# danieljfarrell/pvtrace

Hardware: AMD Instinct MI355X
Metric: photons/sec on 5x5x1 cm Lumogen-F-Red LSC (higher is better)
Workload: dtype f64

## Files before the change

### __graft_entry__.py

```python
import os
import subprocess
import sys

ROOT = os.path.dirname(os.path.abspath(__file__))
CSRC = os.path.join(ROOT, "pvtrace_amd", "csrc")
LIB = os.path.join(CSRC, "libpvtrace_hip.so")
HIPCC_FLAGS = [
    "--offload-arch=gfx950", "-O3", "-std=c++17",
    "-ffp-contract=off", "-fno-fast-math",
    "-munsafe-fp-atomics",
    "-mllvm", "-disable-machine-licm",
    "-fno-unroll-loops",
    "-fPIC", "-shared",
]


def _stale(target, sources):
    if not os.path.exists(target):
        return True
    t = os.path.getmtime(target)
    return any(os.path.getmtime(s) > t for s in sources if os.path.exists(s))


def build(force=False):
# ... 49 lines not shown
    for block in notes.split("- .agpr_count:")[1:]:
        name = re.search(r"\.name:\s+(\S+)", block).group(1)
        out[name] = {k: int(v) for k, v in re.findall(r"\.(sgpr_spill_count|vgpr_count|vgpr_spill_count|"
                                                      r"private_segment_fixed_size):\s+(\d+)", block)}
        out[name]["text_bytes"] = size.get(name, 0)
    return out


def code_hash(lib=LIB):
    import hashlib
    import tempfile

    llvm = "/opt/rocm/lib/llvm/bin"
    with tempfile.TemporaryDirectory() as tmp:
        fat, co, text = (os.path.join(tmp, f) for f in ("fat.bin", "k.co", "text.bin"))
        subprocess.check_call([os.path.join(llvm, "llvm-objcopy"), "-O", "binary", "--only-section=.hip_fatbin", lib, fat])
        subprocess.check_call([os.path.join(llvm, "clang-offload-bundler"), "--unbundle", "--type=o", f"--input={fat}",
                               "--targets=hipv4-amdgcn-amd-amdhsa--gfx950", f"--output={co}"],
                              stdout=subprocess.DEVNULL, stderr=subprocess.DEVNULL)
        subprocess.check_call([os.path.join(llvm, "llvm-objcopy"), "-O", "binary", "--only-section=.text", co, text])
        return hashlib.sha256(open(text, "rb").read()).hexdigest()[:16]


def check_kernel_budgets():
    meta = kernel_metadata()
    head = [m for n, m in meta.items() if "trace_kernel_w4ILb0ELi1ELi1ELb0E" in n]
    problems = []
    if head:
        m = head[0]
        if m["vgpr_count"] > 128 or m["vgpr_spill_count"] or m["private_segment_fixed_size"] > 320:
            problems.append(f"headline variant needs {m['vgpr_count']} vector registers, {m['vgpr_spill_count']} spilled, "
                            f"{m['private_segment_fixed_size']} B of scratch (budget: <= 128, 0, a call frame of <= 320 B)")
        if m["sgpr_spill_count"] > 60:
            problems.append(f"headline variant spills {m['sgpr_spill_count']} scalar registers (budget: <= 60)")
        if m["text_bytes"] > 58 * 1024:
            problems.append(f"headline variant is {m['text_bytes']} bytes of code (budget: 58 KB of the 64 KB instruction cache)")
    for n, m in meta.items():
        if "trace_kernel_gridILb0E" in n and "ELi1E" in n and (m["vgpr_spill_count"] or m["private_segment_fixed_size"] > 320):
            problems.append(f"grid-walk variant {n} uses scratch memory ({m['vgpr_spill_count']} spilled registers, "
                            f"{m['private_segment_fixed_size']} B)")
    for p in problems:
        print("=" * 100 + f"\n[build] WARNING: kernel budget exceeded -- {p}\n" + "=" * 100, file=sys.stderr)
    return problems


def smoke():
    if ROOT not in sys.path:
        sys.path.insert(0, ROOT)
    import numpy as np

    from oracle import oracle
    from pvtrace_amd.engine import _kernel, compile_scene
    from pvtrace_amd.engine.emit import emit_bundle
    from benchmarks.configs import cfg2_lsc

    scene = cfg2_lsc()
    compiled = compile_scene(scene)
    pos, dirs, wl, _ = emit_bundle(scene, 4096, seed=1)
    gpu = _kernel.trace_bundle(compiled, pos, dirs, wl, 7, 1000, 64, 0, 1, 1)
    cpu = oracle.trace_bundle(compiled, pos, dirs, wl, 7, 1000, 64, 0, 1, 1,
                              math_mode=oracle.MATH_PORTABLE)
    for key in cpu:
        if key == "rec_sums":
# ... 12 lines not shown
```

### include/pvtrace_hip.h

```cpp
#ifndef PVTRACE_HIP_H
#define PVTRACE_HIP_H

#include <stdint.h>

#ifdef __cplusplus
extern "C" {
#endif

#define PVT_ABI_VERSION 13

#define PVT_MAX_NODES 128
#define PVT_MAX_RECORDERS 256
#define PVT_MAX_HITS 512

enum {
    PVT_EV_GENERATE = 0, PVT_EV_REFLECT = 1, PVT_EV_TRANSMIT = 2, PVT_EV_ABSORB = 3,
    PVT_EV_NONRADIATIVE = 4, PVT_EV_SCATTER = 5, PVT_EV_EMIT = 6, PVT_EV_EXIT = 7,
    PVT_EV_REACT = 8, PVT_EV_KILL = 9,
    PVT_EV_DETECT = 10
};
enum { PVT_GEOM_BOX = 0, PVT_GEOM_SPHERE = 1, PVT_GEOM_CYLINDER = 2, PVT_GEOM_MESH = 3,
       PVT_GEOM_FRUSTUM = 4 };
enum { PVT_SURF_FRESNEL = 0, PVT_SURF_NULL = 1 };
enum { PVT_COMP_ABSORBER = 0, PVT_COMP_SCATTERER = 1, PVT_COMP_LUMINOPHORE = 2, PVT_COMP_REACTOR = 3 };
// ... 366 lines not shown
                           const PvtRays* rays, const PvtTraceParams* params,
                           const PvtTallies* tallies, const PvtEventLog* log,
                           const int* devices, int n_devices, double* kernel_ms);

int pvt_last_multi_reduce(void);

int pvt_shard_range(int64_t n_rays, int shard, int n_shards, int64_t align, int64_t* start, int64_t* stop);

int pvt_emit_device(PvtScene* scene, const PvtTraceParams* params, double* position,
                    double* direction, double* wavelength, void* stream);

int pvt_selftest_math(int fn, const double* x_host, double* y_host, int64_t n, int device);

int pvt_scene_counters(PvtScene* scene, uint64_t* out, int reset);

int pvt_scene_clock(PvtScene* scene, uint64_t* out);

int pvt_scene_launch_span(PvtScene* scene, void* stream, uint64_t* out);

int pvt_scene_launch_info(PvtScene* scene, int32_t* grid, int32_t* block, int32_t* lds_bytes);

enum { PVT_VARIANT_LEAN = 0, PVT_VARIANT_W4 = 1, PVT_VARIANT_GRID = 2, PVT_VARIANT_ROUGH = 3, PVT_VARIANT_MESH = 4 };
int pvt_scene_variant(PvtScene* scene);
int pvt_scene_lean_check(const PvtSceneTables* tables, const PvtIndexTables* index_tables, const PvtPhaseTables* phase_tables,
                         const PvtSurfaceTables* surface_tables, const PvtFieldTables* field_tables,
                         const PvtMapTables* map_tables, int32_t* lean);

int pvt_mesh_bvh_check(const PvtSceneTables* tables, int32_t node, int32_t* n_bvh_nodes,
                       int32_t* n_leaves, int32_t* depth);

int pvt_node_grid_plan(const PvtSceneTables* tables, int32_t* dims, double* lo, double* cell, double* guard,
                       int32_t* odd, uint64_t* masks, int64_t masks_cap);

#ifdef __cplusplus
}
#endif
#endif
```

### pvtrace_amd/csrc/pvt_trace.hip

```cpp
#include <hip/hip_runtime.h>

#include <cmath>
#include <cstdio>
#include <cstdlib>
#include <algorithm>
#include <atomic>
#include <cstring>
#include <chrono>
#include <dlfcn.h>
#include <string>
#include <thread>
#include <type_traits>
#include <mutex>
#include <vector>

#include "../../include/pvtrace_hip.h"
#include "pvt_math.h"
#include "pvt_bvh.h"

#include "pvt_trace_kernel.h"

namespace {

thread_local std::string g_error;
// ... 74 lines not shown
    };
    std::vector<Carry> carry;
    std::vector<double*> emit_pool;
    std::vector<size_t> emit_pool_bytes;
    std::vector<double*> origin_store;
    std::vector<size_t> origin_store_bytes;
    unsigned int carry_cap = 0;
    int num_cu = 0;
    int last_grid = 0, last_lds = 0;
    size_t lds_limit = 0;
    int lazy_root = 0;
    double lazy_k = 0.0;
    bool exit_observed = false;
    bool grid = false;
    int grid_dims[3] = {0, 0, 0};
    bool fuse_exit = false;
    bool hist_reads_position = false;
    bool hist_reads_counter = false;
    int origin_mask = 0;
    int counting() const { return hist_reads_counter ? 2 : d_cd ? 1 : 0; }
    bool lean_ok = false;
    bool lean_even = false;
    int last_variant = -1;
};

extern "C" {

int pvt_abi_version(void) { return PVT_ABI_VERSION; }
const char* pvt_last_error(void) { return g_error.c_str(); }

int pvt_device_count(void) {
    int n = 0;
    if (hipGetDeviceCount(&n) != hipSuccess) return 0;
    return n;
}

int pvt_scene_set_emitter(PvtScene* s, const PvtEmitterTables* e) {
    if (!s || !e || e->n_lights <= 0) return fail(PVT_ERR_INVALID, "bad emitter");
    HIP_TRY(hipSetDevice(s->device));
    std::vector<double> ed;
    std::vector<int> ei;
    EmitOff o{};
    const int Lt = e->n_lights;
    o.wl_value = push(ed, e->wl_value, Lt);
    o.pos_param = push(ed, e->pos_param, (size_t)Lt * 3);
    o.dir_param = push(ed, e->dir_param, Lt);
// ... 130 lines not shown
    const size_t small_bytes = (size_t)s->nd_small * 8 + (size_t)((s->ni_small + 1) & ~1) * 4;
    if (acc_bytes + tq_bytes + tab_bytes <= budget && !force) lp.tab = Tab::Lds;
    else if (s->meshq == 0 && acc_bytes + tq_bytes + small_bytes <= 40 * 1024 && acc_bytes + tq_bytes + small_bytes <= budget &&
             !(force && force[0] == 'g')) lp.tab = Tab::Heads;
    size_t lds = acc_bytes + tq_bytes + (lp.tab == Tab::Lds ? tab_bytes : lp.tab == Tab::Heads ? small_bytes : 0);
    lp.bins_in_lds = (lds + bins_bytes <= budget) ? 1 : 0;
    if (lp.bins_in_lds) lds += bins_bytes;
    const size_t xw = 14 + (s->n_rec <= 64 ? 1 : 4) + (record ? 1 : 0) + (s->counting() ? 2 : 0) + (s->origin_mask ? kOriginWords : 0);
    const size_t xbytes = (size_t)kXSlots * xw * 8;
    if (s->meshq == 0 && lds + xbytes <= 40 * 1024 && lds + xbytes <= lds_limit) {
        lp.xslots = kXSlots;
        lds += xbytes;
    }
    lp.total = lp.bytes = (lds + 15) & ~(size_t)15;
    if (s->meshq) {
        lp.meshq_off = (int)lp.total;
        lp.total += (size_t)s->meshq * kBlock * 4;
        lp.top_off = (int)lp.total;
        lp.total += (size_t)s->top_n * sizeof(pvt::BvhNode);
    }
    return lp;
}

struct Variant { int family; bool record; Tab tab; int seenw; bool emit, mesh, grid, even, align; };
Variant choose_variant(const PvtScene* s, const LdsPlan& lp, bool record, bool emit) {
    Variant v{};
    v.record = record; v.emit = emit; v.tab = lp.tab;
    v.seenw = s->n_rec <= 64 ? 1 : 4;
    v.mesh = s->d_bvh != nullptr;
    v.grid = lp.tab == Tab::Lds && s->lay.grid_d >= 0 && !v.mesh;
    const bool extension = s->has_frustum || s->rough_d >= 0 || s->d_fd || s->d_md || s->d_cd || s->cabs_d >= 0 || s->counting() || s->origin_mask || s->pd_d >= 0 || s->al_d >= 0;
    const bool lean = lp.tab == Tab::Lds && s->lean_ok && v.seenw == 1;
    v.align = s->al_d >= 0;
    v.family = extension ? PVT_VARIANT_ROUGH : v.mesh ? PVT_VARIANT_MESH : v.grid ? PVT_VARIANT_GRID : lean ? PVT_VARIANT_LEAN : PVT_VARIANT_W4;
    v.even = v.family == PVT_VARIANT_LEAN && s->lean_even;
    return v;
}

using Kernel = void (*)(KArgs);
template <class F> Kernel with_bool(bool b, F f) { return b ? f(std::true_type{}) : f(std::false_type{}); }
template <class F> Kernel with_tab(Tab t, F f) {
    return t == Tab::Lds ? f(std::integral_constant<int, 1>{}) : t == Tab::Heads ? f(std::integral_constant<int, 2>{}) : f(std::integral_constant<int, 0>{});
}

#ifndef PVT_DEV_VARIANTS
#define PVT_DEV_VARIANTS 0
#endif
Kernel kernel_of(const Variant& v) {
    return with_bool(v.record, [&](auto record) { return with_bool(v.emit, [&](auto emit) { return with_bool(v.seenw == 4, [&](auto wide) {
    return with_tab(v.tab, [&](auto tab) -> Kernel {
        constexpr bool R = decltype(record)::value, E = decltype(emit)::value;
        constexpr int W = decltype(wide)::value ? 4 : 1, T = decltype(tab)::value, dev = PVT_DEV_VARIANTS;
        constexpr bool narrow = T == 1 && W == 1 && !E;
        constexpr bool has_rough = dev == 0;
        constexpr bool has_mesh = T != 2 && (dev == 0 || (dev == 2 && narrow));
        constexpr bool has_grid = T == 1 && (dev == 0 || (dev == 1 && narrow));
        constexpr bool has_lean = T == 1 && W == 1 && (dev == 0 || (dev == 1 && narrow && !R));
        constexpr bool has_w4 = dev == 0 || (dev == 1 && narrow);
        switch (v.family) {
        case PVT_VARIANT_ROUGH:
            if constexpr (has_rough) {
                if (v.align) {
                    if constexpr (T == 1) if (v.grid) return trace_kernel_rough_grid<R, W, E, kExtAligned>;
                    if constexpr (T != 2) if (v.mesh) return trace_kernel_rough<R, T, W, E, true, kExtAligned>;
                    if (!v.mesh) return trace_kernel_rough_w4<R, T, W, E, kExtAligned>;
                    break;
                }
                if constexpr (T == 1) if (v.grid) return trace_kernel_rough_grid<R, W, E>;
                if constexpr (T != 2) if (v.mesh) return trace_kernel_rough<R, T, W, E, true>;
                if (!v.mesh) return trace_kernel_rough_w4<R, T, W, E>;
            }
            break;
        case PVT_VARIANT_MESH:
            if constexpr (has_mesh) return trace_kernel<R, T, W, E, true>;
            break;
        case PVT_VARIANT_GRID:
            if constexpr (has_grid) return trace_kernel_grid<R, W, E>;
            break;
        case PVT_VARIANT_LEAN:
            if constexpr (has_lean) { if (v.even) return trace_kernel_lean_w4<R, E, true>; return trace_kernel_lean_w4<R, E, false>; }
            break;
        case PVT_VARIANT_W4:
            if constexpr (has_w4) return trace_kernel_w4<R, T, W, E>;
            break;
        }
        return nullptr;
    }); }); }); });
}

int check_carried(const PvtScene::Carry& carry, const PvtTraceParams* p) {
    if (p->record_every > 0 || p->tally_bundle > 0)
        return fail(PVT_ERR_INVALID, "photons parked by the previous launch on this stream (PVT_FLAG_CARRY_OUT) are waiting: "
                                     "finish them with a plain tally launch (n_rays may be 0) first");
    if (p->maxsteps != carry.maxsteps || p->emit_method != carry.emit_method)
        return fail(PVT_ERR_INVALID, "photons parked by the previous launch on this stream were traced with maxsteps " +
                                     std::to_string(carry.maxsteps) + ", emit_method " + std::to_string(carry.emit_method) +
                                     "; this launch asks for " + std::to_string(p->maxsteps) + ", " + std::to_string(p->emit_method) +
                                     ": finish them under their own rules first (a launch with n_rays = 0 and the old values), or drop "
                                     "them with pvt_scene_carry_discard");
    return PVT_OK;
}

// ... 156 lines not shown
    a.top_off = lp.top_off; a.top_n = s->top_n; a.bvh_top = s->d_bvh_top;
    if (a.bvh && lp.total > s->lds_limit) return fail(PVT_ERR_INVALID, "mesh staging exceeds LDS");

    const long long grid = size_grid(s, p, carry_in ? carry.bound : 0, n_sets, a);
    s->last_grid = (int)grid;
    s->last_lds = (int)lp.total;
    bool carry_out = (p->flags & PVT_FLAG_CARRY_OUT) != 0 && !record && !n_sets;
    if ((carry_in || carry_out) && (rc = bind_carry(s, carry, blocks, grid, carry_in, &carry_out, a)) != PVT_OK) return rc;

#if PVT_TIMELINE
    if (getenv("PVT_TIMELINE_FILE")) {
        if (!g_timeline) { (void)hipMalloc(&g_timeline, kTlBytes); (void)hipMemset(g_timeline, 0, kTlBytes); }
        const int from = getenv("PVT_TIMELINE_FROM") ? atoi(getenv("PVT_TIMELINE_FROM")) : 0;
        const int k = g_tl_launch++ - from;
        if (k >= 0 && k < kTlLaunches && grid <= kTlWgs) {
            a.timeline = g_timeline + (size_t)k * kTlWgs * kWaves * 8;
            g_tl_grid[k] = (int)grid; g_tl_n[k] = p->n_rays;
        }
    }
#endif
    const bool emit = rays == nullptr && s->d_ed != nullptr;
    if (emit && (rc = grow_emit_pool(s, (size_t)slot, grid, st, a)) != PVT_OK) return rc;
    if (s->origin_mask && (rc = grow_origin_store(s, (size_t)slot, grid, st, a)) != PVT_OK) return rc;
    const Variant v = choose_variant(s, lp, record, emit);
    s->last_variant = v.family;
    hipError_t e = hipErrorNotSupported;
    if (const Kernel kernel = kernel_of(v)) {
        hipLaunchKernelGGL(kernel, dim3((unsigned)grid), dim3(kBlock), lp.total, st, a);
        e = hipGetLastError();
    }
    if (e != hipSuccess) return fail(PVT_ERR_HIP, std::string("trace_kernel launch: ") + hipGetErrorString(e));
    if (!n_sets) carry.phase = (carry.phase + 1) % 3;
    if (carry_in || carry_out) {
        carry.pending = carry_out;
        carry.bound = carry_out ? grid * kBlock : 0;
        carry.maxsteps = p->maxsteps;
        carry.emit_method = p->emit_method;
        carry.parity ^= 1;
    }
#if PVT_STATS
    dump_stats(a, st);
#endif
    return PVT_OK;
}

#if PVT_TIMELINE
void timeline_dump() {
    const char* path = getenv("PVT_TIMELINE_FILE");
// ... 396 lines not shown
    size_t k = 0;
    {
        std::lock_guard<std::mutex> lock(s->slot_mutex);
        while (k < s->slot_of.size() && s->slot_of[k] != reinterpret_cast<hipStream_t>(stream)) k++;
        if (k == s->slot_of.size()) return fail(PVT_ERR_INVALID, "no launch on this stream yet");
    }
    HIP_TRY(hipStreamSynchronize(reinterpret_cast<hipStream_t>(stream)));
    HIP_TRY(hipMemcpy(out, s->d_stamp + 2 * k, 16, hipMemcpyDeviceToHost));
    return PVT_OK;
}

int pvt_scene_launch_info(PvtScene* s, int32_t* grid, int32_t* block, int32_t* lds_bytes) {
    if (!s) return fail(PVT_ERR_INVALID, "null scene");
    if (grid) *grid = s->last_grid;
    if (block) *block = kBlock;
    if (lds_bytes) *lds_bytes = s->last_lds;
    return PVT_OK;
}

int pvt_scene_variant(PvtScene* s) {
    if (!s) return fail(PVT_ERR_INVALID, "null scene");
    if (s->last_variant >= 0) return s->last_variant;
    return choose_variant(s, plan_lds(s, false), false, false).family;
}

int pvt_scene_lean_check(const PvtSceneTables* t, const PvtIndexTables* x, const PvtPhaseTables* ph, const PvtSurfaceTables* rs,
                         const PvtFieldTables* fr, const PvtMapTables* mp, int32_t* lean) {
    if (!t || !lean) return fail(PVT_ERR_INVALID, "null argument");
    if (t->n_nodes <= 0 || t->n_nodes > PVT_MAX_NODES || t->n_recorders > PVT_MAX_RECORDERS) return fail(PVT_ERR_INVALID, "bad argument");
    PackedScene packed;
    const int rc = pack_scene({t, x, ph, rs, fr, mp, nullptr, nullptr, nullptr, kKnowsOrigin}, &packed);
    if (rc != PVT_OK) return rc;
    *lean = packed.lean_ok ? (packed.lean_even ? 2 : 1) : 0;
    return PVT_OK;
}

int pvt_mesh_bvh_check(const PvtSceneTables* t, int32_t node, int32_t* n_bvh_nodes, int32_t* n_leaves,
                       int32_t* depth_out) {
    if (!t || node < 0 || node >= t->n_nodes || t->geom_type[node] != PVT_GEOM_MESH)
        return fail(PVT_ERR_INVALID, "not a mesh node");
    const int f0 = t->mesh_face_start[node], fc = t->mesh_face_count[node];
    if (fc <= 0 || f0 < 0 || f0 + fc > t->n_mesh_faces) return fail(PVT_ERR_INVALID, "mesh face range out of bounds");
    std::vector<pvt::BvhNode> nodes;
    std::vector<pvt::MeshTri> tris;
    double centre[3];
    const int root = pvt::BvhBuilder(t->mesh_vertices, t->mesh_faces, t->mesh_normals, nodes, tris).add_mesh(f0, fc, centre);
// ... 653 lines not shown
```

### pvtrace_amd/csrc/pvt_trace_kernel.h

```cpp
#pragma once
constexpr int kMeshWaves = 4;
#ifndef PVT_STATS
#define PVT_STATS 0
#endif
#ifndef PVT_TIMELINE
#define PVT_TIMELINE 0
#endif

namespace {

constexpr int kBlock = 256;
constexpr int kChunk = 64;
constexpr int kEndClaim = 64;
constexpr int kClaim = kChunk;
constexpr int kWaves = kBlock / 64;
constexpr int kCursorSlots = 64;
constexpr int kMaxSets = 1024;
constexpr int kRecPlain = 1 << 30;
constexpr int kTallyQ = 64;
constexpr int kXSlots = 72;
enum { CTL_EXHAUSTED = 0, CTL_DONE = 1, CTL_IN = 2, CTL_LIVE = 6, CTL_COUNT = 16, CTL_CLOCK = 22, CTL_WORDS = 26 };
constexpr double kEps = 2.220446049250313e-13;
constexpr double kAlphaZero = 1e-8;
constexpr double kCcm = 2.99792458e10;
// ... 743 lines not shown
    else if (dt == PVT_DIR_ISOTROPIC) ld = sample_phase(PVT_PHASE_ISOTROPIC, 0.0, rng);
    else if (dt == PVT_DIR_HG) ld = sample_phase(PVT_PHASE_HG, prm, rng);
    else if (dt == PVT_DIR_LAMBERTIAN) {
        double p1 = rng_uniform(rng), p2 = rng_uniform(rng);
        ld = lambert_direction(p1, p2);
    }
    const double* m = ed + E.l2w + li * 16;
    pos.x = m[0] * lp.x + m[1] * lp.y + m[2] * lp.z + m[3];
    pos.y = m[4] * lp.x + m[5] * lp.y + m[6] * lp.z + m[7];
    pos.z = m[8] * lp.x + m[9] * lp.y + m[10] * lp.z + m[11];
    dir.x = m[0] * ld.x + m[1] * ld.y + m[2] * ld.z;
    dir.y = m[4] * ld.x + m[5] * ld.y + m[6] * ld.z;
    dir.z = m[8] * ld.x + m[9] * ld.y + m[10] * ld.z;
}

__device__ __attribute__((noinline)) void emit_chunk(const KArgs* A, unsigned long long gi, double* pool) {
    V3 ep, ed;
    double ew;
    emit_one(*A, gi, ep, ed, ew);
    pool[0] = ep.x; pool[64] = ep.y; pool[128] = ep.z;
    pool[192] = ed.x; pool[256] = ed.y; pool[320] = ed.z;
    pool[384] = ew;
}

__global__ void __launch_bounds__(kBlock) emit_kernel(KArgs A, double* opos, double* odir, double* owl) {
    unsigned int i = blockIdx.x * kBlock + threadIdx.x;
    if (i >= A.n_rays) return;
    V3 p, d;
    double wl;
    emit_one(A, A.ray_offset + i, p, d, wl);
    opos[i * 3] = p.x; opos[i * 3 + 1] = p.y; opos[i * 3 + 2] = p.z;
    odir[i * 3] = d.x; odir[i * 3 + 1] = d.y; odir[i * 3 + 2] = d.z;
    owl[i] = wl;
}

__global__ void __launch_bounds__(kBlock) math_kernel(int fn, const double* x, double* y, long long n) {
    long long i = (long long)blockIdx.x * kBlock + threadIdx.x;
    if (i >= n) return;
    double v = x[i], r;
    switch (fn) {
        case 0: r = pvt_log(v); break;
        case 1: r = pvt_sin(v); break;
        case 2: r = pvt_cos(v); break;
        case 3: r = pvt_asin(v); break;
        case 4: r = pvt_acos(v); break;
        case 5: r = pvt_sqrt(v); break;
// ... 194 lines not shown
    }
    unsigned long long* const out_distinct = reinterpret_cast<unsigned long long*>(A.rec_distinct) + (long long)set * A.set_stride_i;
    unsigned long long* const out_crossings = reinterpret_cast<unsigned long long*>(A.rec_crossings) + (long long)set * A.set_stride_i;
    unsigned long long* const out_bins = reinterpret_cast<unsigned long long*>(A.rec_bins) + (long long)set * A.set_stride_i;
    double* const out_sums = A.rec_sums + (long long)set * A.set_stride_d;
    for (int i = lane; i < A.n_rec; i += 64) {
        const unsigned long long c = acc_cross[i];
        const unsigned int d = acc_distinct[i];
        if (c) atomicAdd(out_crossings + i, c);
        if (d) atomicAdd(out_distinct + i, (unsigned long long)d);
    }
    for (int i = lane; i < A.n_rec * 8; i += 64) {
        double v = acc_sums[i];
        if (v != 0.0) atomicAdd(out_sums + i, v);
    }
    if (A.bins_in_lds)
        for (int i = lane; i < A.total_bins; i += 64) {
            unsigned int v = acc_bins[i];
            if (v) atomicAdd(out_bins + i, (unsigned long long)v);
        }
}

template <bool RECORD, int TAB_LDS, int SEENW, bool EMIT, bool MESH, bool GRID = false, bool TAIL = false, int ROUGH = 0,
          int LEAN = 0>
__device__ __forceinline__ void trace_body(const KArgs& A, int tail_total = 0, unsigned int tail_lds = 0u) {
    static_assert(!LEAN || (!MESH && !GRID && !ROUGH && TAB_LDS == 1 && SEENW == 1), "the lean variants: plain scenes only");
    extern __shared__ double smem_of_kernel[];
    double* const smem = TAIL ? (double*)(__attribute__((address_space(3))) double*)(unsigned long long)tail_lds
                              : (double*)smem_of_kernel;
    constexpr int kAbsKind = LEAN == kLeanEven ? kInterpEven : LEAN ? kInterpNoHist : kInterpAny;
    constexpr int kCdfKind = LEAN == kLeanEven ? kInterpByGuide : LEAN ? kInterpNoHist : kInterpAny;
    auto held = [](int v) __attribute__((always_inline)) -> int {
        if constexpr (TAIL) asm volatile("" : "+s"(v));
        return v;
    };
    const int k_root = held(A.root), k_maxsteps = held(A.maxsteps), k_nodes = held(A.n_nodes);
#if PVT_TIMELINE
    unsigned long long tl_t[6] = {(unsigned long long)wall_clock64(), 0, 0, 0, 0, 0};
    unsigned long long tl_iters = 0;
    const unsigned long long tl_c0 = __builtin_readcyclecounter();
#endif
    Lay L = A.lay;
    if constexpr (TAIL) {
        L.comp_d = held(L.comp_d); L.rec_d = held(L.rec_d); L.hist_d = held(L.hist_d); L.coat_d = held(L.coat_d);
        L.comp_i = held(L.comp_i); L.rec_i = held(L.rec_i); L.hist_i = held(L.hist_i); L.coat_i = held(L.coat_i);
        L.cand_i = held(L.cand_i); L.cand_list = held(L.cand_list); L.crit_d = held(L.crit_d); L.ccrit_d = held(L.ccrit_d);
        L.grid_d = held(L.grid_d); L.rot_d = held(L.rot_d); L.ncls_d = held(L.ncls_d); L.n_cls = held(L.n_cls);
    }
    enum { UF_COATED = 0, UF_FUSE_EXIT, UF_CRIT, UF_HAS_REC, UF_TQ_POS, UF_BINS_LDS, UF_EMIT_FULL, UF_EMIT_KT, UF_LAZY1, UF_LAZY2, UF_BY_NODE,
// ... 231 lines not shown
#define PVT_MARK(k) do { unsigned long long now_ = __builtin_readcyclecounter(); if (ws & WS_SOLO) st_t[k] += now_ - st_mark; st_mark = now_; } while (0)
    unsigned long long st_c[8] = {0, 0, 0, 0, 0, 0, 0, 0};
    unsigned long long st_g[4] = {0, 0, 0, 0};
#define PVT_COUNT(k, pred) do { unsigned long long b_ = __ballot(pred); if (!(ws & WS_EXHAUSTED)) st_c[k] += __popcll(b_); } while (0)
#else
#define PVT_MARK(k) do {} while (0)
#define PVT_COUNT(k, pred) do {} while (0)
#endif
    const unsigned int wgs_in_set = A.set_size ? (unsigned int)A.wgs_per_set : gridDim.x;
    const unsigned int waves_in_set = wgs_in_set * kWaves;
    const unsigned int wave_in_set = (blockIdx.x - set * (A.set_size ? (unsigned int)A.wgs_per_set : 0u)) * kWaves +
                                     (unsigned int)__builtin_amdgcn_readfirstlane((int)(threadIdx.x >> 6));
    const unsigned int w_first = wave_in_set * (unsigned int)kClaim;
    unsigned int w_next = w_first, w_end = w_first, w_base = 0;
    unsigned int w_claim_end = w_first < n_local ? (n_local - w_first < (unsigned int)kClaim ? n_local : w_first + kClaim) : w_first;
    unsigned int c_next = 0, c_end = 0;
    enum { WS_EXHAUSTED = 1, WS_COUNTED = 2, WS_REGIME = 4, WS_SOLO = 8, WS_CARRY_IN = 16, WS_C_FIRST = 32 };
    unsigned int ws = WS_C_FIRST | ((!RECORD && (A.carry_flags & 1) != 0) ? WS_CARRY_IN : 0u);
    const bool seed_pool = A.xslots * (14 + SEENW) >= kWaves * 4 * 64;
    const int pool_at = __builtin_amdgcn_readfirstlane((int)(threadIdx.x >> 6)) * 4 * 64;
    const int wave = __builtin_amdgcn_readfirstlane((int)(threadIdx.x >> 6));
    int members = 0, parity = 0;
    int tail_n = 0;
    constexpr bool kTailCall = !TAIL && !MESH && !(GRID && RECORD);

    auto tally_flush = [&]() {
        if (lane < tq_n) {
            const int r = tq_r[lane];
            const double q_wl = tq_d[lane], q_angle = pvt_acos(tq_d[kTallyQ + lane]);
            const double q_duration = tq_d[2 * kTallyQ + lane], q_travelled = tq_d[3 * kTallyQ + lane];
            const int ri = L.rec_i + r * RI;
            atomicAdd(&acc_distinct[r], 1u);
            double* sp = acc_sums + r * 8;
            atomicAdd(&sp[0], q_wl); atomicAdd(&sp[1], q_wl * q_wl);
            atomicAdd(&sp[2], q_angle); atomicAdd(&sp[3], q_angle * q_angle);
            atomicAdd(&sp[4], q_duration); atomicAdd(&sp[5], q_duration * q_duration);
            atomicAdd(&sp[6], q_travelled); atomicAdd(&sp[7], q_travelled * q_travelled);
            const int h0 = T.iv(ri + RI_HSTART), h1 = h0 + T.iv(ri + RI_HN);
            for (int h = h0; h < h1; h++) {
                const int hi_ = L.hist_i + h * HI, hd_ = L.hist_d + h * HD;
                const int pa = T.iv(hi_ + HI_PA), pb = T.iv(hi_ + HI_PB);
                const int na = T.iv(hi_ + HI_NA), nb = T.iv(hi_ + HI_NB);
                auto prop = [&](int pr) -> double {
                    if (pr < 4) return pr == 0 ? q_wl : pr == 1 ? q_angle : pr == 2 ? q_duration : q_travelled;
                    if constexpr (ROUGH) {
                        if (pr >= 10)
                            return tq_d[tq_count_at + ((uf(UF_TQ_COUNT) ? 1 : 0) + __builtin_popcount(origin_mask() & ((1u << (pr - 10)) - 1u))) * kTallyQ + lane];
// ... 118 lines not shown
                unsigned int b = w_end;
                if (b >= w_claim_end) {
                    const unsigned int claim = (n_local - w_claim_end > 2u * waves_in_set * (unsigned int)kClaim || w_claim_end > n_local)
                                                   ? (unsigned int)kClaim : (unsigned int)kEndClaim;
                    unsigned int c = 0;
                    if (lane == 0) c = atomicAdd(cursor, claim);
                    c = __builtin_amdgcn_readfirstlane(c) + waves_in_set * (unsigned int)kClaim;
                    if (c >= n_local) { ws |= WS_EXHAUSTED; break; }
                    b = c;
                    w_claim_end = (n_local - c < claim) ? n_local : c + claim;
                }
                w_next = b;
                w_end = (w_claim_end - b < (unsigned int)kChunk) ? w_claim_end : b + kChunk;
                w_base = b;
                if constexpr (EMIT) {
                    const __attribute__((address_space(4))) KArgs* ak =
                        (const __attribute__((address_space(4))) KArgs*)__builtin_amdgcn_kernarg_segment_ptr();
                    asm volatile("" : "+s"(ak));
                    unsigned int lane_here = (unsigned int)lane;
                    asm volatile("" : "+v"(lane_here));
                    if (b + lane_here < w_end) {
                        double* pool = ak->emit_pool + ((unsigned long long)blockIdx.x * kWaves + (unsigned long long)wave) * (7 * 64) + lane_here;
                        const unsigned long long gi_ = A.ray_offset + (unsigned long long)ray_lo + (unsigned long long)b + (unsigned long long)lane_here;
                        emit_chunk((const KArgs*)ak, gi_, pool);
                    }
                }
                if (seed_pool) {
                    unsigned int lane_here = (unsigned int)lane;
                    asm volatile("" : "+v"(lane_here));
                    unsigned long long st = A.seed + (unsigned long long)ray_lo + (unsigned long long)b + (unsigned long long)lane_here;
#pragma unroll
                    for (int k = 0; k < 4; k++) {
                        xbuf[pool_at + k * 64 + lane] = splitmix64(st);
                        __builtin_amdgcn_sched_barrier(0);
                    }
                }
            }
            unsigned int avail = w_end - w_next;
            unsigned int rank = rank_in(need);
            unsigned int want = __popcll(need);
            if (!alive && rank < avail) {
                const unsigned int il = w_next + rank;
                const unsigned int i = ray_lo + il;
                if constexpr (EMIT) {
                    const __attribute__((address_space(4))) KArgs* ak =
                        (const __attribute__((address_space(4))) KArgs*)__builtin_amdgcn_kernarg_segment_ptr();
                    asm volatile("" : "+s"(ak));
// ... 22 lines not shown
                duration = 0.0;
                count = 0;
                source = -1;
                nev = 0;
                if constexpr (ROUGH) {
                    if (uf(UF_CAPTURE)) gidx = A.ray_offset + (unsigned long long)i;
                    if (uf(UF_COUNT)) hcount = 0ull;
                    if (uf(UF_ORIGIN)) origin_put(wl, pos.x, pos.y, pos.z);
                }
#pragma unroll
                for (int w = 0; w < SEENW; w++) seen.w[w] = 0ull;
                alive = true;
                if constexpr (RECORD) {
                    rec_slot = -1;
                    if (A.record_every > 0 && (long long)i % A.record_every == 0) rec_slot = (int)((long long)i / A.record_every);
                    log_row<RECORD, TAIL>(A, rec_slot, nev, PVT_EV_GENERATE, -1, -1, -1, -1, source, pos, dir, false,
                                    pos, wl, travelled, duration);
                }
            }
            w_next += (want < avail) ? want : avail;
            need = __ballot(!alive);
        }
        if constexpr (!RECORD) {
            if ((ws & WS_EXHAUSTED) && (A.carry_flags & 2)) {
                const unsigned long long live_mask = __ballot(alive);
                if (live_mask != 0ull) {
                    const __attribute__((address_space(4))) KArgs* ak =
                        (const __attribute__((address_space(4))) KArgs*)__builtin_amdgcn_kernarg_segment_ptr();
                    asm volatile("" : "+s"(ak));
                    unsigned int b = 0;
                    if (lane == 0) b = atomicAdd(cursor + 2, (unsigned int)__popcll(live_mask));
                    b = __builtin_amdgcn_readfirstlane(b);
                    const unsigned int at = b + rank_in(live_mask);
                    if (alive && at < ak->carry_cap) {
                        unsigned long long* dst = ak->carry_out + (unsigned long long)at * ((ROUGH && uf(UF_COUNT) ? kCarryStrideCount : kCarryStride) + (ROUGH && uf(UF_ORIGIN) ? kOriginWords : 0));
                        dst[0] = pvt_d2u(pos.x); dst[1] = pvt_d2u(pos.y); dst[2] = pvt_d2u(pos.z);
                        dst[3] = pvt_d2u(dir.x); dst[4] = pvt_d2u(dir.y); dst[5] = pvt_d2u(dir.z);
                        dst[6] = pvt_d2u(wl); dst[7] = pvt_d2u(travelled); dst[8] = pvt_d2u(duration);
                        dst[9] = rng.s0; dst[10] = rng.s1; dst[11] = rng.s2; dst[12] = rng.s3;
                        dst[13] = (unsigned long long)(unsigned int)count | ((unsigned long long)(unsigned int)source << 32);
#pragma unroll
                        for (int w = 0; w < SEENW; w++) dst[kCarryBase + w] = seen.w[w];
                        if constexpr (ROUGH) {
                            if (uf(UF_CAPTURE)) dst[kCarryStride] = gidx;
                            if (uf(UF_COUNT)) dst[kCarryStride + 1] = hcount;
                            if (uf(UF_ORIGIN)) {
                                const int co = origin_cat();
                                const double* o = origin_slot();
#pragma unroll
                                for (int k = 0; k < kOriginWords; k++) dst[co + k] = pvt_d2u(o[k]);
                            }
                        }
                    }
                    alive = false;
                }
            }
        }
        if ((ws & (WS_EXHAUSTED | WS_COUNTED)) == WS_EXHAUSTED) {
            ws |= WS_COUNTED;
            if (lane == 0) atomicAdd(&ctl[CTL_EXHAUSTED], 1);
        }
        if (!(ws & WS_REGIME)) {
            if (__ballot(alive) == 0ull) break;
            if (A.xslots > 0 && (ws & (WS_EXHAUSTED | WS_SOLO)) == WS_EXHAUSTED &&
                __builtin_amdgcn_readfirstlane(__hip_atomic_load(&ctl[CTL_EXHAUSTED], __ATOMIC_RELAXED, __HIP_MEMORY_SCOPE_WORKGROUP)) == kWaves) {
                ws |= WS_REGIME;
                if (lane == 0) ctl[CTL_IN + wave] = 1;
                __syncthreads();
                members = __builtin_amdgcn_readfirstlane((ctl[CTL_IN] ? 1 : 0) | (ctl[CTL_IN + 1] ? 2 : 0) | (ctl[CTL_IN + 2] ? 4 : 0) |
                                                         (ctl[CTL_IN + 3] ? 8 : 0));
            }
        }
        if (ws & WS_REGIME) {
            const unsigned long long live_mask = __ballot(alive);
            const int live = __popcll(live_mask);
            int* live_tab = ctl + CTL_LIVE + parity * kWaves;
            parity ^= 1;
            if (lane == 0) live_tab[wave] = live;
            __syncthreads();
            int l[kWaves], total = 0, nw = 0, before = 0, pos_in_set = 0;
// ... 88 lines not shown
                    for (int w = 0; w < SEENW; w++) seen.w[w] = xbuf[(14 + w) * X + slot];
                    if constexpr (RECORD) {
                        const unsigned long long rn_ = xbuf[(14 + SEENW) * X + slot];
                        rec_slot = (int)(unsigned int)rn_;
                        nev = (int)(unsigned int)(rn_ >> 32);
                    }
                    if constexpr (ROUGH) {
                        if (uf(UF_CAPTURE)) gidx = xbuf[kXWords * X + slot];
                        if (uf(UF_COUNT)) hcount = xbuf[(kXWords + 1) * X + slot];
                        if (uf(UF_ORIGIN)) {
                            const int xo = origin_xat();
                            origin_put(pvt_u2d(xbuf[xo * X + slot]), pvt_u2d(xbuf[(xo + 1) * X + slot]), pvt_u2d(xbuf[(xo + 2) * X + slot]),
                                       pvt_u2d(xbuf[(xo + 3) * X + slot]));
                        }
                    }
                }
                int kept = 0, m2 = 0;
#pragma unroll
                for (int w = 0; w < kWaves; w++)
                    if (((members >> w) & 1) && kept < keep) { m2 |= 1 << w; kept += 1; }
                members = m2;
                if (keep == 1) ws = (ws & ~(unsigned int)WS_REGIME) | WS_SOLO;
            }
        }
        }
#if PVT_STATS
        {
            unsigned long long live = __popcll(__ballot(alive));
            st_iters += 1; st_lane_steps += live;
            if (ws & WS_EXHAUSTED) { st_drain_iters += 1; st_drain_lane_steps += live; }
        }
#endif

        c_iters += 1u;
#if PVT_TIMELINE
        if (tl_iters == 0) tl_t[2] = wall_clock64();
        if ((ws & WS_EXHAUSTED) && tl_t[3] == 0) tl_t[3] = wall_clock64();
        tl_iters += 1;
#endif
        PVT_MARK(0);
        PVT_COUNT(0, alive);
        int ev_kind = -1, ev_hit = -1, ev_container = -1, ev_adjacent = -1, ev_component = -1;
        bool ev_normal = false, terminal = false;
        int t_sel = -1, t_node = -1;
        bool t_normal = false;
        double t_cos = 1.0;
// ... 1245 lines not shown
__global__ void __launch_bounds__(kBlock) __attribute__((amdgpu_waves_per_eu(4, 4))) trace_kernel_w4(KArgs A) {
    trace_body<RECORD, TAB_LDS, SEENW, EMIT, false>(A);
}
template <bool RECORD, int SEENW, bool EMIT>
__global__ void __launch_bounds__(kBlock) __attribute__((amdgpu_waves_per_eu(4, 4))) trace_kernel_grid(KArgs A) {
    trace_body<RECORD, 1, SEENW, EMIT, false, true>(A);
}
template <bool RECORD, int TAB_LDS, int SEENW, bool EMIT, bool MESH, int EXT = kExtRough>
__global__ void __launch_bounds__(kBlock) __attribute__((amdgpu_waves_per_eu(kMeshWaves, kMeshWaves))) trace_kernel_rough(KArgs A) {
    trace_body<RECORD, TAB_LDS, SEENW, EMIT, MESH, false, false, EXT>(A);
}
template <bool RECORD, int TAB_LDS, int SEENW, bool EMIT, int EXT = kExtRough>
__global__ void __launch_bounds__(kBlock) __attribute__((amdgpu_waves_per_eu(4, 4))) trace_kernel_rough_w4(KArgs A) {
    trace_body<RECORD, TAB_LDS, SEENW, EMIT, false, false, false, EXT>(A);
}
template <bool RECORD, int SEENW, bool EMIT, int EXT = kExtRough>
__global__ void __launch_bounds__(kBlock) __attribute__((amdgpu_waves_per_eu(4, 4))) trace_kernel_rough_grid(KArgs A) {
    trace_body<RECORD, 1, SEENW, EMIT, false, true, false, EXT>(A);
}
template <bool RECORD, bool EMIT, bool EVEN>
__global__ void __launch_bounds__(kBlock) __attribute__((amdgpu_waves_per_eu(4, 4))) trace_kernel_lean_w4(KArgs A) {
    trace_body<RECORD, 1, 1, EMIT, false, false, false, false, EVEN ? kLeanEven : kLeanSearched>(A);
}

}
```

### pvtrace_amd/engine/native.py

```python
import ctypes as C
import os
import threading

import numpy as np

_HERE = os.path.dirname(os.path.abspath(__file__))
LIB_PATH = os.environ.get(
    "PVT_LIB", os.path.join(os.path.dirname(_HERE), "csrc", "libpvtrace_hip.so"))

_p_i32 = C.POINTER(C.c_int32)
_p_f64 = C.POINTER(C.c_double)
_p_i64 = C.POINTER(C.c_int64)
_p_u8 = C.POINTER(C.c_uint8)


class EngineUnavailableError(RuntimeError):
    """The HIP engine cannot run here (library not built, or no MI355X visible)."""


def _same_names(fields):
    return {name: (name, np.int32 if ctype is _p_i32 else np.float64) for name, ctype in fields if ctype in (_p_i32, _p_f64)}


class PvtSceneTables(C.Structure):
# ... 381 lines not shown
        "pvt_scene_carry_discard": ([vp, vp], C.c_int),
        "pvt_scene_trim": ([vp], C.c_int),
        "pvt_last_multi_reduce": ([], C.c_int),
        "pvt_unpack_records_device": (
            [C.POINTER(PvtEventRecords), C.c_int64, C.c_int32, C.POINTER(PvtEventLog), C.c_int, vp], C.c_int),
        "pvt_trace_bundle": (
            [C.POINTER(PvtSceneTables), C.POINTER(PvtEmitterTables), C.POINTER(PvtRays),
             C.POINTER(PvtTraceParams), C.POINTER(PvtTallies), C.POINTER(PvtEventLog), C.c_int,
             C.POINTER(C.c_double)], C.c_int),
        "pvt_trace_bundle_multi": (
            [C.POINTER(PvtSceneTables), C.POINTER(PvtEmitterTables), C.POINTER(PvtRays),
             C.POINTER(PvtTraceParams), C.POINTER(PvtTallies), C.POINTER(PvtEventLog), C.POINTER(C.c_int),
             C.c_int, C.POINTER(C.c_double)], C.c_int),
        "pvt_release_cached_memory": ([], None),
        "pvt_shard_range": ([C.c_int64, C.c_int, C.c_int, C.c_int64, C.POINTER(C.c_int64), C.POINTER(C.c_int64)], C.c_int),
        "pvt_emit_device": ([vp, C.POINTER(PvtTraceParams), vp, vp, vp, vp], C.c_int),
        "pvt_selftest_math": ([C.c_int, vp, vp, C.c_int64, C.c_int], C.c_int),
        "pvt_mesh_bvh_check": (
            [C.POINTER(PvtSceneTables), C.c_int32, C.POINTER(C.c_int32), C.POINTER(C.c_int32),
             C.POINTER(C.c_int32)], C.c_int),
        "pvt_scene_launch_info": (
            [vp, C.POINTER(C.c_int32), C.POINTER(C.c_int32), C.POINTER(C.c_int32)], C.c_int),
        "pvt_scene_variant": ([vp], C.c_int),
        "pvt_scene_lean_check": (scene_inputs(LEAN_CHECK_TABLES) + [C.POINTER(C.c_int32)], C.c_int),
        "pvt_scene_counters": ([vp, C.POINTER(C.c_uint64), C.c_int], C.c_int),
        "pvt_scene_clock": ([vp, C.POINTER(C.c_uint64)], C.c_int),
        "pvt_scene_launch_span": ([vp, vp, C.POINTER(C.c_uint64)], C.c_int),
        "pvt_node_grid_plan": (
            [C.POINTER(PvtSceneTables), C.POINTER(C.c_int32), C.POINTER(C.c_double), C.POINTER(C.c_double),
             C.POINTER(C.c_double), C.POINTER(C.c_int32), C.POINTER(C.c_uint64), C.c_int64], C.c_int),
    }
    for name, count in CREATION_ENTRIES.items():
        sigs[name] = (scene_inputs(count) + [C.c_int, C.POINTER(vp)], C.c_int)
    for name in names:
        argtypes, restype = sigs[name]
        fn = getattr(lib, name)
        fn.argtypes = argtypes
        fn.restype = restype
    return sigs


ABI_SYMBOLS = (
    "pvt_abi_version", "pvt_last_error", "pvt_device_count", "pvt_scene_create",
    "pvt_scene_set_emitter", "pvt_scene_destroy", "pvt_trace_device", "pvt_trace_bundle",
    "pvt_emit_device", "pvt_selftest_math", "pvt_scene_launch_info", "pvt_mesh_bvh_check",
    "pvt_trace_bundle_multi", "pvt_shard_range", "pvt_trace_device_records", "pvt_unpack_records_device",
    "pvt_scene_carry_pending", "pvt_last_multi_reduce", "pvt_node_grid_plan", "pvt_scene_carry_discard", "pvt_scene_trim",
    "pvt_scene_counters", "pvt_scene_clock", "pvt_scene_launch_span", "pvt_release_cached_memory",
    "pvt_scene_create_ex", "pvt_scene_create_phase", "pvt_scene_create_rough", "pvt_scene_create_field",
    "pvt_scene_create_maps", "pvt_scene_map_slots", "pvt_scene_variant", "pvt_scene_lean_check",
    "pvt_scene_create_capture", "pvt_scene_capture_rows", "pvt_trace_device_capture", "pvt_scene_create_absorb",
    "pvt_scene_create_origin", "pvt_scene_create_pattern", "pvt_scene_create_aligned",
)
VARIANT_NAMES = ("lean", "w4", "grid", "rough", "mesh")

_lib = None
ABI_VERSION = 13
FLAG_NO_LOG_PREFILL = 1
FLAG_CARRY_OUT = 2


def library_built():
    return os.path.exists(LIB_PATH)


def _preload_torch_hip_runtime():
    import importlib.util

    try:
        spec = importlib.util.find_spec("torch")
    except (ImportError, ValueError):
        spec = None
    if spec is None or not spec.origin:
        return None
    path = os.path.join(os.path.dirname(spec.origin), "lib", "libamdhip64.so")
    if not os.path.exists(path):
        return None
# ... 160 lines not shown

        torch.cuda.synchronize(self.device)
        out = (C.c_uint64 * 2)()
        check(self.lib.pvt_scene_clock(self.handle, out), "pvt_scene_clock")
        cycles, ticks = int(out[0]), int(out[1])
        return {"shader_cycles": cycles, "ticks_100mhz": ticks, "shader_clock_mhz": 100.0 * cycles / ticks if ticks else 0.0}

    def launch_span_ms(self, stream=None):
        import torch

        if stream is None:
            stream = torch.cuda.current_stream(self.device).cuda_stream
        out = (C.c_uint64 * 2)()
        check(self.lib.pvt_scene_launch_span(self.handle, C.c_void_p(stream), out), "pvt_scene_launch_span")
        return (int(out[1]) - int(out[0])) * 1e-5

    def launch_info(self):
        g, b, l = C.c_int32(), C.c_int32(), C.c_int32()
        check(self.lib.pvt_scene_launch_info(self.handle, C.byref(g), C.byref(b), C.byref(l)),
              "pvt_scene_launch_info")
        variant = int(self.lib.pvt_scene_variant(self.handle))
        if variant < 0:
            check(variant, "pvt_scene_variant")
        return {"grid": g.value, "block": b.value, "lds_bytes": l.value, "variant": VARIANT_NAMES[variant]}

    def new_tallies(self, sets=1, captures=True):
        import torch

        from pvtrace_amd.engine.tally_set import TallySet

        return TallySet(self.compiled, torch.device("cuda", self.device), sets=sets, captures=captures)

    def new_event_log(self, n_rays, record_every, max_events):
        import torch

        dev = torch.device("cuda", self.device)
        nrec = num_recorded(n_rays, record_every)
        rows = nrec * max_events
        return {"counts": torch.empty(max(nrec, 1), dtype=torch.int32, device=dev),
                "rows": torch.empty((max(rows, 1), RECORD_WORDS), dtype=torch.int64, device=dev)}

    def new_event_columns(self, n_rays, record_every, max_events):
        import torch

        dev = torch.device("cuda", self.device)
        nrec = num_recorded(n_rays, record_every)
        rows = nrec * max_events
# ... 140 lines not shown
```

Baseline: 4.052 billion.

## Add parking lean kernel entry for carry-out tally launches at higher occupancy

Adds a new lean-family kernel entry (trace_kernel_lean_park) that is used for tally launches with carry-out enabled. Once the ray supply is exhausted it parks live photons for the next launch and exits, instead of running the tail, regime-switching and tail-call logic. Emission goes through a noinline helper, and the kernel targets five waves per EU instead of four. The aim is to cut register pressure and drain-phase inefficiency to gain occupancy, at the cost of more carry-over work and possible spills if the tighter register budget is exceeded.

```diff
diff --git a/__graft_entry__.py b/__graft_entry__.py
--- a/__graft_entry__.py
+++ b/__graft_entry__.py
@@ -95,8 +95,9 @@
         return hashlib.sha256(open(text, "rb").read()).hexdigest()[:16]
 
 
-def check_kernel_budgets():
-    meta = kernel_metadata()
+def check_kernel_budgets(meta=None):
+    if meta is None:
+        meta = kernel_metadata()
     head = [m for n, m in meta.items() if "trace_kernel_w4ILb0ELi1ELi1ELb0E" in n]
     problems = []
     if head:
@@ -112,6 +113,12 @@
         if "trace_kernel_gridILb0E" in n and "ELi1E" in n and (m["vgpr_spill_count"] or m["private_segment_fixed_size"] > 320):
             problems.append(f"grid-walk variant {n} uses scratch memory ({m['vgpr_spill_count']} spilled registers, "
                             f"{m['private_segment_fixed_size']} B)")
+    lean_frame = max([m["private_segment_fixed_size"] for n, m in meta.items() if "trace_kernel_lean_w4ILb0E" in n], default=0)
+    for n, m in meta.items():
+        if "trace_kernel_lean_park" in n and (m["vgpr_count"] > 96 or m["vgpr_spill_count"] > 2 or
+                                              m["private_segment_fixed_size"] > lean_frame):
+            problems.append(f"parking entry {n} needs {m['vgpr_count']} vector registers, {m['vgpr_spill_count']} spilled, "
+                            f"{m['private_segment_fixed_size']} B of scratch (budget: <= 96, <= 2, <= {lean_frame} B)")
     for p in problems:
         print("=" * 100 + f"\n[build] WARNING: kernel budget exceeded -- {p}\n" + "=" * 100, file=sys.stderr)
     return problems
diff --git a/include/pvtrace_hip.h b/include/pvtrace_hip.h
--- a/include/pvtrace_hip.h
+++ b/include/pvtrace_hip.h
@@ -412,6 +412,8 @@
 
 enum { PVT_VARIANT_LEAN = 0, PVT_VARIANT_W4 = 1, PVT_VARIANT_GRID = 2, PVT_VARIANT_ROUGH = 3, PVT_VARIANT_MESH = 4 };
 int pvt_scene_variant(PvtScene* scene);
+enum { PVT_ENTRY_USUAL = 0, PVT_ENTRY_PARK = 1 };
+int pvt_scene_entry(PvtScene* scene);
 int pvt_scene_lean_check(const PvtSceneTables* tables, const PvtIndexTables* index_tables, const PvtPhaseTables* phase_tables,
                          const PvtSurfaceTables* surface_tables, const PvtFieldTables* field_tables,
                          const PvtMapTables* map_tables, int32_t* lean);
diff --git a/pvtrace_amd/csrc/pvt_trace.hip b/pvtrace_amd/csrc/pvt_trace.hip
--- a/pvtrace_amd/csrc/pvt_trace.hip
+++ b/pvtrace_amd/csrc/pvt_trace.hip
@@ -120,6 +120,7 @@
     bool lean_ok = false;
     bool lean_even = false;
     int last_variant = -1;
+    bool last_park = false;
 };
 
 extern "C" {
@@ -296,8 +297,8 @@
     return lp;
 }
 
-struct Variant { int family; bool record; Tab tab; int seenw; bool emit, mesh, grid, even, align; };
-Variant choose_variant(const PvtScene* s, const LdsPlan& lp, bool record, bool emit) {
+struct Variant { int family; bool record; Tab tab; int seenw; bool emit, mesh, grid, even, align, park; };
+Variant choose_variant(const PvtScene* s, const LdsPlan& lp, bool record, bool emit, bool carry_out = false) {
     Variant v{};
     v.record = record; v.emit = emit; v.tab = lp.tab;
     v.seenw = s->n_rec <= 64 ? 1 : 4;
@@ -308,6 +309,7 @@
     v.align = s->al_d >= 0;
     v.family = extension ? PVT_VARIANT_ROUGH : v.mesh ? PVT_VARIANT_MESH : v.grid ? PVT_VARIANT_GRID : lean ? PVT_VARIANT_LEAN : PVT_VARIANT_W4;
     v.even = v.family == PVT_VARIANT_LEAN && s->lean_even;
+    v.park = v.family == PVT_VARIANT_LEAN && !record && carry_out;
     return v;
 }
 
@@ -352,6 +354,7 @@
             if constexpr (has_grid) return trace_kernel_grid<R, W, E>;
             break;
         case PVT_VARIANT_LEAN:
+            if constexpr (has_lean && !R) if (v.park) { if (v.even) return trace_kernel_lean_park<E, true>; return trace_kernel_lean_park<E, false>; }
             if constexpr (has_lean) { if (v.even) return trace_kernel_lean_w4<R, E, true>; return trace_kernel_lean_w4<R, E, false>; }
             break;
         case PVT_VARIANT_W4:
@@ -554,8 +557,9 @@
     const bool emit = rays == nullptr && s->d_ed != nullptr;
     if (emit && (rc = grow_emit_pool(s, (size_t)slot, grid, st, a)) != PVT_OK) return rc;
     if (s->origin_mask && (rc = grow_origin_store(s, (size_t)slot, grid, st, a)) != PVT_OK) return rc;
-    const Variant v = choose_variant(s, lp, record, emit);
+    const Variant v = choose_variant(s, lp, record, emit, carry_out);
     s->last_variant = v.family;
+    s->last_park = v.park;
     hipError_t e = hipErrorNotSupported;
     if (const Kernel kernel = kernel_of(v)) {
         hipLaunchKernelGGL(kernel, dim3((unsigned)grid), dim3(kBlock), lp.total, st, a);
@@ -998,6 +1002,11 @@
     if (!s) return fail(PVT_ERR_INVALID, "null scene");
     if (s->last_variant >= 0) return s->last_variant;
     return choose_variant(s, plan_lds(s, false), false, false).family;
+}
+
+int pvt_scene_entry(PvtScene* s) {
+    if (!s) return fail(PVT_ERR_INVALID, "null scene");
+    return s->last_park ? PVT_ENTRY_PARK : PVT_ENTRY_USUAL;
 }
 
 int pvt_scene_lean_check(const PvtSceneTables* t, const PvtIndexTables* x, const PvtPhaseTables* ph, const PvtSurfaceTables* rs,
diff --git a/pvtrace_amd/csrc/pvt_trace_kernel.h b/pvtrace_amd/csrc/pvt_trace_kernel.h
--- a/pvtrace_amd/csrc/pvt_trace_kernel.h
+++ b/pvtrace_amd/csrc/pvt_trace_kernel.h
@@ -789,6 +789,14 @@
     pool[192] = ed.x; pool[256] = ed.y; pool[320] = ed.z;
     pool[384] = ew;
 }
+__device__ __attribute__((noinline)) void emit_chunk_park(const KArgs* A, unsigned long long gi, double* pool) {
+    V3 ep, ed;
+    double ew;
+    emit_one(*A, gi, ep, ed, ew);
+    pool[0] = ep.x; pool[64] = ep.y; pool[128] = ep.z;
+    pool[192] = ed.x; pool[256] = ed.y; pool[320] = ed.z;
+    pool[384] = ew;
+}
 
 __global__ void __launch_bounds__(kBlock) emit_kernel(KArgs A, double* opos, double* odir, double* owl) {
     unsigned int i = blockIdx.x * kBlock + threadIdx.x;
@@ -1029,9 +1037,10 @@
 }
 
 template <bool RECORD, int TAB_LDS, int SEENW, bool EMIT, bool MESH, bool GRID = false, bool TAIL = false, int ROUGH = 0,
-          int LEAN = 0>
+          int LEAN = 0, bool PARK = false>
 __device__ __forceinline__ void trace_body(const KArgs& A, int tail_total = 0, unsigned int tail_lds = 0u) {
     static_assert(!LEAN || (!MESH && !GRID && !ROUGH && TAB_LDS == 1 && SEENW == 1), "the lean variants: plain scenes only");
+    static_assert(!PARK || (LEAN && !RECORD && !TAIL), "the parking form: tally launches of the lean family only");
     extern __shared__ double smem_of_kernel[];
     double* const smem = TAIL ? (double*)(__attribute__((address_space(3))) double*)(unsigned long long)tail_lds
                               : (double*)smem_of_kernel;
@@ -1309,7 +1318,7 @@
     const int wave = __builtin_amdgcn_readfirstlane((int)(threadIdx.x >> 6));
     int members = 0, parity = 0;
     int tail_n = 0;
-    constexpr bool kTailCall = !TAIL && !MESH && !(GRID && RECORD);
+    constexpr bool kTailCall = !TAIL && !MESH && !(GRID && RECORD) && !PARK;
 
     auto tally_flush = [&]() {
         if (lane < tq_n) {
@@ -1474,7 +1483,8 @@
                     if (b + lane_here < w_end) {
                         double* pool = ak->emit_pool + ((unsigned long long)blockIdx.x * kWaves + (unsigned long long)wave) * (7 * 64) + lane_here;
                         const unsigned long long gi_ = A.ray_offset + (unsigned long long)ray_lo + (unsigned long long)b + (unsigned long long)lane_here;
-                        emit_chunk((const KArgs*)ak, gi_, pool);
+                        if constexpr (PARK) emit_chunk_park((const KArgs*)ak, gi_, pool);
+                        else emit_chunk((const KArgs*)ak, gi_, pool);
                     }
                 }
                 if (seed_pool) {
@@ -1543,7 +1553,7 @@
             need = __ballot(!alive);
         }
         if constexpr (!RECORD) {
-            if ((ws & WS_EXHAUSTED) && (A.carry_flags & 2)) {
+            if ((ws & WS_EXHAUSTED) && (PARK || (A.carry_flags & 2))) {
                 const unsigned long long live_mask = __ballot(alive);
                 if (live_mask != 0ull) {
                     const __attribute__((address_space(4))) KArgs* ak =
@@ -1577,6 +1587,10 @@
                 }
             }
         }
+        if constexpr (PARK) {
+            if (ws & WS_EXHAUSTED) break;
+            if (__ballot(alive) == 0ull) break;
+        } else {
         if ((ws & (WS_EXHAUSTED | WS_COUNTED)) == WS_EXHAUSTED) {
             ws |= WS_COUNTED;
             if (lane == 0) atomicAdd(&ctl[CTL_EXHAUSTED], 1);
@@ -1711,6 +1725,7 @@
                 members = m2;
                 if (keep == 1) ws = (ws & ~(unsigned int)WS_REGIME) | WS_SOLO;
             }
+        }
         }
         }
 #if PVT_STATS
@@ -3002,5 +3017,12 @@
 __global__ void __launch_bounds__(kBlock) __attribute__((amdgpu_waves_per_eu(4, 4))) trace_kernel_lean_w4(KArgs A) {
     trace_body<RECORD, 1, 1, EMIT, false, false, false, false, EVEN ? kLeanEven : kLeanSearched>(A);
 }
-
-}
+#ifndef PVT_PARK_WAVES
+#define PVT_PARK_WAVES 5
+#endif
+template <bool EMIT, bool EVEN>
+__global__ void __launch_bounds__(kBlock) __attribute__((amdgpu_waves_per_eu(PVT_PARK_WAVES, PVT_PARK_WAVES))) trace_kernel_lean_park(KArgs A) {
+    trace_body<false, 1, 1, EMIT, false, false, false, false, EVEN ? kLeanEven : kLeanSearched, true>(A);
+}
+
+}
diff --git a/pvtrace_amd/engine/native.py b/pvtrace_amd/engine/native.py
--- a/pvtrace_amd/engine/native.py
+++ b/pvtrace_amd/engine/native.py
@@ -427,6 +427,7 @@
         "pvt_scene_launch_info": (
             [vp, C.POINTER(C.c_int32), C.POINTER(C.c_int32), C.POINTER(C.c_int32)], C.c_int),
         "pvt_scene_variant": ([vp], C.c_int),
+        "pvt_scene_entry": ([vp], C.c_int),
         "pvt_scene_lean_check": (scene_inputs(LEAN_CHECK_TABLES) + [C.POINTER(C.c_int32)], C.c_int),
         "pvt_scene_counters": ([vp, C.POINTER(C.c_uint64), C.c_int], C.c_int),
         "pvt_scene_clock": ([vp, C.POINTER(C.c_uint64)], C.c_int),
@@ -455,9 +456,10 @@
     "pvt_scene_create_ex", "pvt_scene_create_phase", "pvt_scene_create_rough", "pvt_scene_create_field",
     "pvt_scene_create_maps", "pvt_scene_map_slots", "pvt_scene_variant", "pvt_scene_lean_check",
     "pvt_scene_create_capture", "pvt_scene_capture_rows", "pvt_trace_device_capture", "pvt_scene_create_absorb",
-    "pvt_scene_create_origin", "pvt_scene_create_pattern", "pvt_scene_create_aligned",
+    "pvt_scene_create_origin", "pvt_scene_create_pattern", "pvt_scene_create_aligned", "pvt_scene_entry",
 )
 VARIANT_NAMES = ("lean", "w4", "grid", "rough", "mesh")
+ENTRY_NAMES = {"lean": ("trace_kernel_lean_w4", "trace_kernel_lean_park")}
 
 _lib = None
 ABI_VERSION = 13
@@ -664,7 +666,13 @@
         variant = int(self.lib.pvt_scene_variant(self.handle))
         if variant < 0:
             check(variant, "pvt_scene_variant")
-        return {"grid": g.value, "block": b.value, "lds_bytes": l.value, "variant": VARIANT_NAMES[variant]}
+        info = {"grid": g.value, "block": b.value, "lds_bytes": l.value, "variant": VARIANT_NAMES[variant]}
+        entry = int(self.lib.pvt_scene_entry(self.handle))
+        if entry < 0:
+            check(entry, "pvt_scene_entry")
+        if VARIANT_NAMES[variant] in ENTRY_NAMES:
+            info["entry"] = ENTRY_NAMES[VARIANT_NAMES[variant]][entry]
+        return info
 
     def new_tallies(self, sets=1, captures=True):
         import torch
```

After: 4.453 billion (median of 6 runs). 1.1x the previous value.
